# Kotomiya07/kuzushiji-vision

Hardware: AMD Instinct MI355X
Metric: line-images/sec (train) (higher is better)
Workload: dtype bf16; 1 GPU; TrOCR train step: ViT-B/16 (12L/768/12h/3072) on 64x640 crops (S_e=161) + RoBERTa decoder 6L/256/4h/768, V=4300 one-char vocab, labels [B,128], dropout 0.1, clip 1.0, RAdamScheduleFree; BASELINE.json configs[1]; per_gpu_batch=256, global_batch=256, parallelism=dp1

## Files before the change

### include/kzv.h

```cpp
#ifndef KZV_H
#define KZV_H
#include <stddef.h>
#include <stdint.h>

#ifdef __cplusplus
extern "C" {
#endif

#define KZV_OK 0
#define KZV_E_ARG (-1)
#define KZV_E_HIP (-2)
#define KZV_E_STATE (-3)

const char* kzv_last_error(void);
int kzv_version(void);

typedef struct kzv_config {
    int32_t image_h, image_w, patch_h, patch_w, channels;
    int32_t enc_hidden, enc_layers, enc_heads, enc_ffn;
    int32_t dec_hidden, dec_layers, dec_heads, dec_ffn;
    int32_t vocab, max_pos, type_vocab, pad_id;
    float enc_hidden_dropout, enc_attn_dropout, dec_hidden_dropout, dec_attn_dropout;
    float ln_eps;
} kzv_config;
// ... 206 lines not shown
    void* c8; int64_t ldc8;
    const float* c8_qscale; float* c8_amax;
    int32_t M, N, K, n_valid;
    float drop_p; uint32_t drop_key;
    const float* c8_rowq;
} kzv_gemm_nt_fp8_args;
int kzv_gemm_nt_fp8(const kzv_gemm_nt_fp8_args* a, int epilogue, void* stream);
int kzv_quant_rows_fp8(const float* x, int64_t rows, int64_t cols, void* q, float* scale, void* stream);
int kzv_layernorm_fwd_fp8(const float* x, const float* gamma, const float* beta, void* y_bf16, void* y_fp8, float* y_scale,
                          float* stats, int rows, int H, float eps, void* stream);
int kzv_set_fp8(kzv_model* m, int mode);
int kzv_get_fp8(const kzv_model* m);
int kzv_fp8_act_scales(const kzv_model* m, float* d_out, void* stream);

typedef struct kzv_gemm_tn_args {
    const void* P; int64_t ldp;
    const void* Q; int64_t ldq;
    float* OUT; int64_t ldo;
    int32_t Mtok, N, K, n_store;
    float* dbias;
} kzv_gemm_tn_args;
int kzv_gemm_tn(const kzv_gemm_tn_args* a, void* stream);

int kzv_gemm_dgrad_wgrad(const kzv_gemm_nt_args* nt, int epilogue, const kzv_gemm_tn_args* tn, void* stream);
int kzv_set_pair(int on);

int kzv_gemm_nt_f32(const kzv_gemm_nt_args* a, int epilogue, void* stream);
int kzv_gemm_tn_f32(const kzv_gemm_tn_args* a, void* stream);

int kzv_layernorm_fwd(const float* x, const float* gamma, const float* beta, void* y_bf16, float* y_f32,
                      float* stats , int rows, int H, float eps, void* stream);
int kzv_layernorm_bwd(const void* dy, int dy_is_f32, const float* x, const float* stats, const float* gamma,
                      float* dx, int accumulate_dx, float* dgamma, float* dbeta, int rows, int H, void* stream);
typedef struct kzv_ln_fwd_args {
    const float* x; const float* gamma; const float* beta;
    void* y_bf16; float* y_f32;
    float* stats;
    int32_t rows, H, seq, drop_first;
    float eps, drop_p; uint32_t drop_key;
} kzv_ln_fwd_args;
int kzv_ln_fwd_ex(const kzv_ln_fwd_args* a, void* stream);
typedef struct kzv_ln_bwd_args {
    const void* dy; const float* x; const float* stats; const float* gamma;
    float* dx; float* dgamma; float* dbeta;
    void* out16;
    int32_t dy_is_f32, accumulate_dx, rows, H, seq, drop_first;
// ... 150 lines not shown
```

### kuzushiji-vision_amd/csrc/gemm.hip

```cpp
#include "kzv_common.h"
#include "../../include/kzv.h"
#include "kzv_host.h"
#include "gemm_nt.h"
#include "gemm_tn.h"

namespace {

constexpr int BK = 64;
constexpr int STAGE_BYTES = (128 + 128) * BK * 2;
constexpr int NT_LDS = 2 * STAGE_BYTES;

template <int N> __device__ __forceinline__ void wait_vmcnt() {
    if constexpr (N == 0) asm volatile("s_waitcnt vmcnt(0)" ::: "memory");
    else if constexpr (N == 4) asm volatile("s_waitcnt vmcnt(4)" ::: "memory");
    else if constexpr (N == 6) asm volatile("s_waitcnt vmcnt(6)" ::: "memory");
    else if constexpr (N == 8) asm volatile("s_waitcnt vmcnt(8)" ::: "memory");
    else if constexpr (N == 12) asm volatile("s_waitcnt vmcnt(12)" ::: "memory");
    else if constexpr (N == 16) asm volatile("s_waitcnt vmcnt(16)" ::: "memory");
    else static_assert(N == 0, "add the vmcnt literal");
}

template <int EPI, int WM, int WN, int NSTAGE, int KB, bool ASM_DMA>
__global__ __launch_bounds__(WM * WN * 64) void gemm_nt_kernel(const NtParams p) {
    constexpr int BM = WM * 64, BN = WN * 64, NW = WM * WN;
// ... 280 lines not shown
    const bool interior = tnb * 128 + 128 <= p.n_store && tkb * 128 + 128 <= p.K;
    for (int it0 = 0; it0 < 64; it0 += 8) {
        float v[8];
#pragma unroll
        for (int u = 0; u < 8; ++u) {
            const int it = it0 + u;
            const int n = w * 32 + (it >> 1), k = (it & 1) * 64 + lane;
            v[u] = tile[n * 128 + ((((k >> 2) ^ (n & 31)) << 2) | (k & 3))];
        }
#pragma unroll
        for (int u = 0; u < 8; ++u) {
            const int it = it0 + u;
            const int n = w * 32 + (it >> 1), k = (it & 1) * 64 + lane;
            const int gn = tnb * 128 + n, gk = tkb * 128 + k;
            float* o = p.OUT + (int64_t)gn * p.ldo + gk;
            if (interior && p.splits > 1) atomicAdd(o, v[u]);
            else if (gn < p.n_store && gk < p.K) { if (p.splits == 1) *o += v[u]; else atomicAdd(o, v[u]); }
        }
    }
}

__global__ __launch_bounds__(256, 2) void gemm_tn_kernel(const TnParams p) { gemm_tn_body(p, blockIdx.x); }

constexpr int TN_GROUP_MAX = 40;
struct TnGroup { TnParams p[TN_GROUP_MAX]; int start[TN_GROUP_MAX + 1]; int n; };
__global__ __launch_bounds__(256, 2) void gemm_tn_group_kernel(const TnGroup g) {
    int i = 0;
#pragma unroll 1
    while (i + 1 < g.n && (int)blockIdx.x >= g.start[i + 1]) ++i;
    gemm_tn_body(g.p[i], (int)blockIdx.x - g.start[i]);
}

}

static int g_nt_schedule = -1;
static int g_nt_half_mask = -1;
static int nt_schedule() {
    if (g_nt_schedule < 0) {
        g_nt_schedule = kzv_env_int("KZV_NT_FREE", 0) != 0;
        if (kzv_env_int("KZV_NT_HALF", 0)) g_nt_schedule |= 2;
    }
    return g_nt_schedule;
}
static int nt_half_mask() {
    if (g_nt_half_mask < 0) g_nt_half_mask = kzv_env_int("KZV_NT_HALF_EPIS", 0x3f);
    return g_nt_half_mask;
}
extern "C" int kzv_set_nt_schedule(int n) { g_nt_schedule = n < 0 ? -1 : (n & 3); return KZV_OK; }
// ... 126 lines not shown
    if (splits < 1) splits = 1;
    const int chunk_tiles = (tok_tiles + splits - 1) / splits;
    splits = (tok_tiles + chunk_tiles - 1) / chunk_tiles;
    p.splits = splits; p.chunk = chunk_tiles * 64;
    return tiles * splits;
}
static int tn_target() {
    static int target = -1;
    if (target < 0) target = kzv_env_int("KZV_TN_BLOCKS", 512);
    return target;
}

extern "C" int kzv_gemm_tn(const kzv_gemm_tn_args* a, void* stream) {
    TnParams p;
    const int rc = tn_fill(a, p);
    if (rc != KZV_OK) return rc;
    KzvProfScope prof(1, 2.0 * a->Mtok * p.n_store * a->K, (hipStream_t)stream);
    if (kzv_tn256_launch(p, (hipStream_t)stream)) return kzv_check_launch("gemm_tn");
    const int blocks = tn_plan(p, tn_target());
    kzv_launch_lds<gemm_tn_kernel>(dim3(blocks), dim3(256), NT_LDS, (hipStream_t)stream, p);
    return kzv_check_launch("gemm_tn");
}

int kzv_gemm_tn_group(const kzv_gemm_tn_args* a, int n, hipStream_t s) {
    if (n <= 0) return KZV_OK;
    if (n == 1 || n > TN_GROUP_MAX) {
        for (int i = 0; i < n; ++i) { const int rc = kzv_gemm_tn(a + i, s); if (rc != KZV_OK) return rc; }
        return KZV_OK;
    }
    TnGroup g;
    g.n = 0;
    int tiles_total = 0;
    double work = 0;
    for (int i = 0; i < n; ++i) {
        TnParams p;
        const int rc = tn_fill(a + i, p);
        if (rc != KZV_OK) return rc;
        const int t256 = ((p.n_store + 255) / 256) * ((p.K + 255) / 256);
        if (t256 >= 24) { const int r2 = kzv_gemm_tn(a + i, s); if (r2 != KZV_OK) return r2; continue; }
        g.p[g.n++] = p;
        tiles_total += ((p.N + 127) / 128) * ((p.K + 127) / 128);
        work += 2.0 * p.Mtok * p.n_store * p.K;
    }
    if (g.n == 0) return KZV_OK;
    KzvProfScope prof(1, work, s);
    int blocks = 0;
    for (int i = 0; i < g.n; ++i) {
        const int tiles = ((g.p[i].N + 127) / 128) * ((g.p[i].K + 127) / 128);
        const int target = tiles_total >= 256 ? 2 * tn_target() : tn_target();
        int share = (int)((int64_t)target * tiles / tiles_total);
        if (share < tiles) share = tiles;
        g.start[i] = blocks;
        blocks += tn_plan(g.p[i], share);
    }
    g.start[g.n] = blocks;
    kzv_launch_lds<gemm_tn_group_kernel>(dim3(blocks), dim3(256), NT_LDS, s, g);
    return kzv_check_launch("gemm_tn_group");
}
```

### kuzushiji-vision_amd/csrc/gemm_tn.h

```cpp
#pragma once
#include "kzv_common.h"

struct TnParams {
    const bf16_t* P; const bf16_t* Q; float* OUT; const void* zero16;
    int64_t ldp, ldq, ldo;
    int Mtok, N, K, n_store, splits, chunk;
    float* dbias;
};

inline bool tn_dma_offsets_fit(const TnParams& p) {
    return (uint64_t)64 * (uint64_t)p.ldp * 2 + (uint64_t)p.N * 2 <= 0xffffffffull && (uint64_t)64 * (uint64_t)p.ldq * 2 + (uint64_t)p.K * 2 <= 0xffffffffull;
}

int kzv_tn256_launch(const TnParams& p, hipStream_t s);

struct KzvTnFoldScope { explicit KzvTnFoldScope(hipStream_t stream); ~KzvTnFoldScope(); hipStream_t s; };

struct kzv_gemm_nt_args; struct kzv_gemm_tn_args;
int kzv_gemm_pair_launch(const kzv_gemm_nt_args* na, int epilogue, const kzv_gemm_tn_args* ta, hipStream_t s);
```

### kuzushiji-vision_amd/csrc/gemm_tn256.hip

```cpp
#include "kzv_common.h"
#include "../../include/kzv.h"
#include "kzv_host.h"
#include "gemm_tn.h"
#include "gemm_nt.h"
#include "gemm256_common.h"
#include "gemm_nt256p_body.h"
#include <vector>
#include <type_traits>

namespace {

constexpr int HT_BYTES = 64 * 256;
constexpr int BUF_BYTES = 4 * HT_BYTES;
constexpr int LDS_BYTES = 2 * BUF_BYTES;
constexpr int KP0 = 0, KP1 = 1, KQ0 = 2, KQ1 = 3;
#ifndef KZV_TN_F32_PARTIALS
constexpr size_t PART_FLOATS = 32768;
#else
constexpr size_t PART_FLOATS = 65536;
#endif

__global__ __launch_bounds__(512) void gemm_tn256_kernel(const TnParams p, float* part_ws) {
    extern __shared__ __attribute__((aligned(16))) char smem[];
    const int tid = threadIdx.x, lane = tid & 63;
    const int w = __builtin_amdgcn_readfirstlane(tid >> 6);
    const int g = lane >> 4, l15 = lane & 15;
    const int wr = w >> 2, wc = w & 3;
    const int tilesN = (p.N + 255) / 256, tilesK = (p.K + 255) / 256;
    const int per = tilesN * tilesK;
    const int id = xcd_remap(blockIdx.x, per * p.splits);
    const int split = id / per, rem = id - split * per;
    const int tnb = rem / tilesK, tkb = rem - tnb * tilesK;
    const int t_begin = split * p.chunk;
    const int t_end = min(p.Mtok, t_begin + p.chunk);
    const int nt = (t_end - t_begin) >> 6;

    const char* baseP = (const char*)(p.P + (int64_t)t_begin * p.ldp);
    const char* baseQ = (const char*)(p.Q + (int64_t)t_begin * p.ldq);
    const int64_t stepP = 64 * p.ldp * 2, stepQ = 64 * p.ldq * 2;
    unsigned voff[4][2];
#pragma unroll
    for (int j = 0; j < 2; ++j) {
        const int r = (w + 8 * j) * 4 + (lane >> 4);
// ... 115 lines not shown

    stage(0, KP0, 0); stage(0, KQ0, 0); stage(0, KQ1, 0); stage(0, KP1, 0); stage(1, KP0, 1); stage(1, KQ0, 1);
    vmcnt<8>();
    __builtin_amdgcn_s_barrier();
    if (wr == 1) __builtin_amdgcn_s_barrier();
    for (int t = 0; t < nt; t += 2) {
        ktile(I0{}, t);
        if (t + 1 < nt) ktile(I1{}, t + 1);
    }
    if (wr == 0) __builtin_amdgcn_s_barrier();

    if (bias_wave) {
#pragma unroll
        for (int j = 0; j < 8; ++j) {
            float v = bsum[j];
            v += __shfl_xor(v, 16, 64);
            v += __shfl_xor(v, 32, 64);
            const int n = tnb * 256 + (j >> 2) * 128 + wr * 64 + (j & 3) * 16 + l15;
            if (g == 0 && n < p.n_store) atomicAdd(p.dbias + n, v);
        }
    }

    float* tile = (float*)smem;
    float* part = part_ws + (size_t)id * PART_FLOATS;
#pragma unroll
    for (int c = 0; c < 2; ++c) {
        __syncthreads();
#pragma unroll
        for (int j = 0; j < 4; ++j)
#pragma unroll
            for (int i = 0; i < 4; ++i)
#pragma unroll
                for (int r = 0; r < 4; ++r) {
                    const int ln = wr * 64 + j * 16 + 4 * g + r;
                    const int k = (i >> 1) * 128 + wc * 32 + (i & 1) * 16 + l15;
                    tile[ln * 256 + ((((k >> 2) ^ (ln & 31)) << 2) | (k & 3))] = acc[i][c * 4 + j][r];
                }
        __syncthreads();
#pragma unroll
        for (int it = 0; it < 16; ++it) {
            const int ln = w * 16 + it;
            const f32x4 v = *(const f32x4*)(tile + ln * 256 + ((lane ^ (ln & 31)) << 2));
            const int row = c * 128 + ln;
#ifndef KZV_TN_F32_PARTIALS
            typedef __attribute__((ext_vector_type(2))) unsigned u32x2p;
            __builtin_nontemporal_store((u32x2p){pack_bf2(v[0], v[1]), pack_bf2(v[2], v[3])}, (u32x2p*)((bf16_t*)part + row * 256 + lane * 4));
#else
            __builtin_nontemporal_store(v, (f32x4*)(part + row * 256 + lane * 4));
#endif
        }
    }
}

__device__ __forceinline__ void tn256f_body(const TnParams& p, float* const part, const int tnb, const int tkb, const int t_begin, const int nt,
                                            char* const smem) {
    const int tid = threadIdx.x, lane = tid & 63;
    const int w = __builtin_amdgcn_readfirstlane(tid >> 6);
    const int g = lane >> 4, l15 = lane & 15;
    const int wr = w >> 2, wc = w & 3;
    const int tilesK = (p.K + 255) / 256;

    const unsigned ldp2 = (unsigned)p.ldp * 2u, ldq2 = (unsigned)p.ldq * 2u;
    const char* baseP = (const char*)(p.P + (int64_t)t_begin * p.ldp);
    const char* baseQ = (const char*)(p.Q + (int64_t)t_begin * p.ldq);
    const int64_t stepP = 64 * (int64_t)ldp2, stepQ = 64 * (int64_t)ldq2;
    unsigned cP[2], cQ[2];
    {
        const int r = w * 4 + (lane >> 4);
        const int col2 = ((lane & 15) ^ ((r & 7) << 1)) * 16;
#pragma unroll
        for (int h = 0; h < 2; ++h) {
            cP[h] = (unsigned)r * ldp2 + (unsigned)min((tnb * 256 + h * 128) * 2 + col2, (p.N - 8) * 2);
            cQ[h] = (unsigned)r * ldq2 + (unsigned)min((tkb * 256 + h * 128) * 2 + col2, (p.K - 8) * 2);
        }
    }
    const unsigned ldsw = __builtin_amdgcn_readfirstlane((unsigned)(__SIZE_TYPE__)((KZV_LDS char*)smem) + (unsigned)w * 1024u);
// ... 133 lines not shown
            if (g == 0 && n < p.n_store) atomicAdd(p.dbias + n, v);
        }
    }

    float* tile = (float*)smem;
#pragma unroll
    for (int c = 0; c < 2; ++c) {
        __syncthreads();
#pragma unroll
        for (int j = 0; j < 4; ++j)
#pragma unroll
            for (int i = 0; i < 4; ++i)
#pragma unroll
                for (int r = 0; r < 4; ++r) {
                    const int ln = wr * 64 + j * 16 + 4 * g + r;
                    const int k = (i >> 1) * 128 + wc * 32 + (i & 1) * 16 + l15;
                    tile[ln * 256 + ((((k >> 2) ^ (ln & 31)) << 2) | (k & 3))] = acc[i][c * 4 + j][r];
                }
        __syncthreads();
#pragma unroll
        for (int it = 0; it < 16; ++it) {
            const int ln = w * 16 + it;
            const f32x4 v = *(const f32x4*)(tile + ln * 256 + ((lane ^ (ln & 31)) << 2));
            const int row = c * 128 + ln;
#ifndef KZV_TN_F32_PARTIALS
            typedef __attribute__((ext_vector_type(2))) unsigned u32x2p;
            __builtin_nontemporal_store((u32x2p){pack_bf2(v[0], v[1]), pack_bf2(v[2], v[3])}, (u32x2p*)((bf16_t*)part + row * 256 + lane * 4));
#else
            __builtin_nontemporal_store(v, (f32x4*)(part + row * 256 + lane * 4));
#endif
        }
    }
}

__global__ __launch_bounds__(512) void gemm_tn256f_kernel(const TnParams p, float* part_ws) {
    extern __shared__ __attribute__((aligned(16))) char smem[];
    const int tilesN = (p.N + 255) / 256, tilesK = (p.K + 255) / 256;
    const int per = tilesN * tilesK;
    const int id = xcd_remap(blockIdx.x, per * p.splits);
    const int split = id / per, rem = id - split * per;
    const int t_begin = split * p.chunk;
    const int t_end = min(p.Mtok, t_begin + p.chunk);
    tn256f_body(p, part_ws + (size_t)id * PART_FLOATS, rem / tilesK, rem % tilesK, t_begin, (t_end - t_begin) >> 6, smem);
}

struct PairPlan { unsigned short tile[256], split[256], t0[256], cnt[256]; };

template <int EPI>
__global__ __launch_bounds__(512) void gemm_pair_kernel(const NtParams pn, const int tiles, const int tilesN, const int strip_in, const TnParams pt,
                                                        float* part_ws, const int per, const PairPlan plan) {
    extern __shared__ __attribute__((aligned(16))) char smem[];
    nt256p_body<EPI, false>(pn, tiles, tilesN, strip_in, (int)blockIdx.x, (int)gridDim.x, smem);
    const int cnt = plan.cnt[blockIdx.x];
    if (cnt == 0) return;
    __syncthreads();
    const int tile = plan.tile[blockIdx.x], split = plan.split[blockIdx.x];
    const int tilesK = (pt.K + 255) / 256;
    tn256f_body(pt, part_ws + ((size_t)split * per + tile) * PART_FLOATS, tile / tilesK, tile % tilesK, (int)plan.t0[blockIdx.x] * 64, cnt, smem);
}

__global__ __launch_bounds__(256) void gemm_tn256_fold_kernel(const float* part_ws, float* OUT, int64_t ldo, int n_store, int K,
                                                             int tilesK, int per, int splits) {
    const int tile = blockIdx.x >> 6;
    const int row = (blockIdx.x & 63) * 4 + (threadIdx.x >> 6), k4 = (threadIdx.x & 63) * 4;
    const int tnb = tile / tilesK, tkb = tile - tnb * tilesK;
    const int gn = tnb * 256 + row, gk = tkb * 256 + k4;
    if (gn >= n_store || gk >= K) return;
    f32x4 s = (f32x4){0.f, 0.f, 0.f, 0.f};
#ifndef KZV_TN_F32_PARTIALS
    typedef __attribute__((ext_vector_type(2))) unsigned u32x2p;
#pragma unroll 4
    for (int sp = 0; sp < splits; ++sp) {
        const u32x2p u = __builtin_nontemporal_load((const u32x2p*)((const bf16_t*)(part_ws + ((size_t)sp * per + tile) * PART_FLOATS) + row * 256 + k4));
        s[0] += bf2f((bf16_t)(u[0] & 0xffffu)); s[1] += bf2f((bf16_t)(u[0] >> 16)); s[2] += bf2f((bf16_t)(u[1] & 0xffffu)); s[3] += bf2f((bf16_t)(u[1] >> 16));
    }
#else
    const float* src = part_ws + ((size_t)tile * 256 + row) * 256 + k4;
#pragma unroll 4
    for (int sp = 0; sp < splits; ++sp) s += __builtin_nontemporal_load((const f32x4*)(src + (size_t)sp * per * PART_FLOATS));
#endif
    f32x4* o = (f32x4*)(OUT + (int64_t)gn * ldo + gk);
    *o += s;
}

constexpr int TN_REGIONS = 6;
KzvScratch g_tn_buf;
size_t g_tn_region = 0;
float* tn_partials(size_t floats, int region) {
    const size_t stride = floats > g_tn_region ? floats : g_tn_region;
    float* base = (float*)g_tn_buf.get((size_t)TN_REGIONS * stride * sizeof(float));
    if (!base) return nullptr;
    g_tn_region = stride;
    return base + (size_t)region * stride;
}

struct TnFold { const float* ws; float* OUT; int64_t ldo; int n_store, K, tilesK, per, splits, block0; };
struct TnFoldTable { TnFold e[TN_REGIONS - 1]; int n; };
__global__ __launch_bounds__(256) void gemm_tn256_fold_multi_kernel(const TnFoldTable t) {
    int k = 0;
    while (k + 1 < t.n && (int)blockIdx.x >= t.e[k + 1].block0) ++k;
    const TnFold& e = t.e[k];
    const int bid = blockIdx.x - e.block0;
    const int tile = bid >> 6;
    const int row = (bid & 63) * 4 + (threadIdx.x >> 6), k4 = (threadIdx.x & 63) * 4;
    const int tnb = tile / e.tilesK, tkb = tile - tnb * e.tilesK;
    const int gn = tnb * 256 + row, gk = tkb * 256 + k4;
    if (gn >= e.n_store || gk >= e.K) return;
    f32x4 s = (f32x4){0.f, 0.f, 0.f, 0.f};
#ifndef KZV_TN_F32_PARTIALS
    typedef __attribute__((ext_vector_type(2))) unsigned u32x2p;
#pragma unroll 4
    for (int sp = 0; sp < e.splits; ++sp) {
        const u32x2p u = __builtin_nontemporal_load((const u32x2p*)((const bf16_t*)(e.ws + ((size_t)sp * e.per + tile) * PART_FLOATS) + row * 256 + k4));
        s[0] += bf2f((bf16_t)(u[0] & 0xffffu)); s[1] += bf2f((bf16_t)(u[0] >> 16)); s[2] += bf2f((bf16_t)(u[1] & 0xffffu)); s[3] += bf2f((bf16_t)(u[1] >> 16));
    }
#else
    const float* src = e.ws + ((size_t)tile * 256 + row) * 256 + k4;
#pragma unroll 4
    for (int sp = 0; sp < e.splits; ++sp) s += __builtin_nontemporal_load((const f32x4*)(src + (size_t)sp * e.per * PART_FLOATS));
#endif
    f32x4* o = (f32x4*)(e.OUT + (int64_t)gn * e.ldo + gk);
    *o += s;
}
int g_tn_defer = 0;
std::vector<TnFold> g_tn_pending;
int tn_flush(hipStream_t s) {
    if (g_tn_pending.empty()) return KZV_OK;
    TnFoldTable t;
    int blocks = 0;
    for (size_t i = 0; i < g_tn_pending.size(); ++i) { t.e[i] = g_tn_pending[i]; t.e[i].block0 = blocks; blocks += g_tn_pending[i].per * 64; }
    t.n = (int)g_tn_pending.size();
    hipLaunchKernelGGL(gemm_tn256_fold_multi_kernel, dim3(blocks), dim3(256), 0, s, t);
    g_tn_pending.clear();
    return kzv_check_launch("gemm_tn256_fold");
}

int g_tn_schedule = -1;
int tn_schedule() {
    if (g_tn_schedule < 0) g_tn_schedule = kzv_env_int("KZV_TN_FREE", 1) != 0;
    return g_tn_schedule;
}
int tn256_min_tiles() {
    static int v = -1;
    if (v < 0) v = kzv_env_int("KZV_TN256_MIN_TILES", 9);
    return v;
}

}

int kzv_tn256_launch(const TnParams& p0, hipStream_t s) {
    const int tiles = ((p0.N + 255) / 256) * ((p0.K + 255) / 256);
    const int tok_tiles = p0.Mtok / 64;
    if (tiles < tn256_min_tiles() || p0.Mtok % 64 || tok_tiles < 2 || p0.N < 8 || p0.K < 8) return 0;
    if (!tn_dma_offsets_fit(p0)) return 0;
    TnParams p = p0;
    int cus = kzv_device_cus() - kzv_cu_reserve();
    { const int g = kzv_env_int("KZV_TN_CUS", 0); if (g > 0 && g < cus) cus = g; }
    int splits = cus / tiles;
    if (splits > tok_tiles / 8) splits = tok_tiles / 8;
    if (splits < 1) splits = 1;
    int chunk_tiles = (tok_tiles + splits - 1) / splits;
    if (chunk_tiles < 2) chunk_tiles = 2;
    splits = (tok_tiles + chunk_tiles - 1) / chunk_tiles;
    if (tok_tiles - (splits - 1) * chunk_tiles < 2) return 0;
    p.splits = splits; p.chunk = chunk_tiles * 64;
    if (p.K % 4 || p.ldo % 4 || ((uintptr_t)p.OUT & 15)) return 0;
    const size_t need = (size_t)tiles * splits * PART_FLOATS;
    const bool deferred = g_tn_defer > 0;
    bool same_out = false;
    for (const TnFold& e : g_tn_pending) same_out |= e.OUT == p.OUT;
    if (deferred && ((int)g_tn_pending.size() == TN_REGIONS - 1 || need > g_tn_region || same_out)) {
        if (tn_flush(s) != KZV_OK) return 0;
    }
    float* ws = tn_partials(need, deferred ? 1 + (int)g_tn_pending.size() : 0);
    if (!ws) return 0;
    if (tn_schedule()) kzv_launch_lds<gemm_tn256f_kernel>(dim3(tiles * splits), dim3(512), LDS_BYTES, s, p, ws);
    else kzv_launch_lds<gemm_tn256_kernel>(dim3(tiles * splits), dim3(512), LDS_BYTES, s, p, ws);
    if (deferred) {
        g_tn_pending.push_back(TnFold{ws, p.OUT, p.ldo, p.n_store, p.K, (p.K + 255) / 256, tiles, splits, 0});
        return 1;
    }
    hipLaunchKernelGGL(gemm_tn256_fold_kernel, dim3(tiles * 64), dim3(256), 0, s, ws, p.OUT, p.ldo, p.n_store, p.K,
                       (p.K + 255) / 256, tiles, splits);
    return 1;
}

int kzv_nt_params(const kzv_gemm_nt_args* a, int epilogue, NtParams* out);

namespace {
int g_pair = -1;
int pair_enabled() {
    if (g_pair < 0) g_pair = kzv_env_int("KZV_PAIR", 0) != 0;
    return g_pair;
}
double pair_ratio(int nk, int epilogue) {
    static int ov = -2;
    if (ov == -2) ov = kzv_env_int("KZV_PAIR_R", -1);
    const double drain = (epilogue == KZV_EPI_DGELU || epilogue == KZV_EPI_RESID) ? 5.0 : 2.5;
    const double r = 0.6 * (nk * 1.45 + drain) / 1.55;
    return ov >= 0 ? r * ov * 0.01 / 0.6 : r;
}
}

int kzv_gemm_pair_launch(const kzv_gemm_nt_args* na, int epilogue, const kzv_gemm_tn_args* ta, hipStream_t s) {
    if (!pair_enabled() || kzv_cu_reserve() != 0 || !tn_schedule() || kzv_device_cus() != 256) return 0;
    if (epilogue != KZV_EPI_BF16 && epilogue != KZV_EPI_F32 && epilogue != KZV_EPI_DGELU && epilogue != KZV_EPI_RESID) return 0;
    NtParams pn;
    if (kzv_nt_params(na, epilogue, &pn) != KZV_OK) return 0;
// ... 31 lines not shown
    std::vector<int> t0((size_t)tilesNw * S), cnt((size_t)tilesNw * S);
    for (int tn = 0; tn < tilesNw; ++tn) {
        double csum = 0;
        for (int sp = 0; sp < S; ++sp) csum += cg[(size_t)tn * S + sp];
        const double level = (stages + r * csum) / S;
        double acc = 0; int prev = 0;
        for (int sp = 0; sp < S; ++sp) {
            double n = level - r * cg[(size_t)tn * S + sp];
            if (n < 2) n = 2;
            acc += n;
            int end = sp == S - 1 ? stages : (int)(acc + 0.5);
            const int left = S - 1 - sp;
            if (end > stages - 2 * left) end = stages - 2 * left;
            if (end < prev + 2) end = prev + 2;
            t0[(size_t)tn * S + sp] = prev; cnt[(size_t)tn * S + sp] = end - prev; prev = end;
        }
        if (prev != stages) return 0;
    }
    for (int b = 0; b < nwg; ++b) {
        const int sp = idb[b] / per, tl = idb[b] % per; const size_t gi = (size_t)(tl / tilesKw) * S + sp;
        plan.tile[b] = (unsigned short)tl; plan.split[b] = (unsigned short)sp; plan.t0[b] = (unsigned short)t0[gi]; plan.cnt[b] = (unsigned short)cnt[gi];
    }
    pt.splits = S; pt.chunk = 0;
    const size_t need = (size_t)per * S * PART_FLOATS;
    const bool deferred = g_tn_defer > 0;
    bool same_out = false;
    for (const TnFold& e : g_tn_pending) same_out |= e.OUT == pt.OUT;
    if (deferred && ((int)g_tn_pending.size() == TN_REGIONS - 1 || need > g_tn_region || same_out)) {
        if (tn_flush(s) != KZV_OK) return 0;
    }
    float* ws = tn_partials(need, deferred ? 1 + (int)g_tn_pending.size() : 0);
    if (!ws) return 0;
    KzvProfScope prof(5, 2.0 * pn.M * pn.n_valid * pn.K + 2.0 * pt.Mtok * pt.N * pt.K, s);
#define KZV_PAIR_CASE(E) case E: kzv_launch_lds<gemm_pair_kernel<E>>(dim3(G), dim3(512), NT256P_LDS_BYTES, s, pn, tiles, tilesN, kzv_nt_strip(), pt, ws, per, plan); break;
    switch (epilogue) {
        KZV_PAIR_CASE(KZV_EPI_BF16) KZV_PAIR_CASE(KZV_EPI_F32) KZV_PAIR_CASE(KZV_EPI_DGELU) KZV_PAIR_CASE(KZV_EPI_RESID)
        default: return 0;
    }
#undef KZV_PAIR_CASE
    if (deferred) g_tn_pending.push_back(TnFold{ws, pt.OUT, pt.ldo, pt.n_store, pt.K, tilesKw, per, S, 0});
    else hipLaunchKernelGGL(gemm_tn256_fold_kernel, dim3(per * 64), dim3(256), 0, s, ws, pt.OUT, pt.ldo, pt.n_store, pt.K, tilesKw, per, S);
    return kzv_check_launch("gemm_pair") == KZV_OK ? 1 : -1;
}

extern "C" int kzv_set_pair(int n) { g_pair = n < 0 ? -1 : (n != 0); return KZV_OK; }
extern "C" int kzv_gemm_dgrad_wgrad(const kzv_gemm_nt_args* na, int epilogue, const kzv_gemm_tn_args* ta, void* stream) {
    if (!na || !ta) return kzv_fail(KZV_E_ARG, "gemm_dgrad_wgrad: null");
// ... 11 lines not shown
```

### kuzushiji-vision_amd/csrc/kzv_kernels.h

```cpp
#pragma once
#include <hip/hip_runtime.h>
#include <stdint.h>
#include "kzv_common.h"

int kzv_ln_fwd_ex(const float* x, const float* gamma, const float* beta, void* y16, float* y32, float* stats,
                  int rows, int H, float eps, int seq, int drop_first, float drop_p, uint32_t drop_key, hipStream_t s,
                  void* y8 = nullptr, float* y8_scale = nullptr);
struct KzvLnBwdF8 { void* out8; float* scale; float* rq; float* rqinv; const float* wnorm; };
int kzv_ln_bwd_ex(const void* dy, int dy_is_f32, const float* x, const float* stats, const float* gamma, float* dx,
                  int accumulate_dx, float* dgamma, float* dbeta, int rows, int H, int seq, int drop_first,
                  float drop_p, uint32_t drop_key, hipStream_t s, bf16_t* out16 = nullptr, float out_drop_p = 0.f,
                  uint32_t out_drop_key = 0, const KzvLnBwdF8* f8 = nullptr);

struct KzvLnDeferScope { explicit KzvLnDeferScope(hipStream_t stream); ~KzvLnDeferScope(); hipStream_t s; };

constexpr int KZV_LN_SLOTS = 32;
float* kzv_ln_partial_region(float* dgamma, float* dbeta, int H, hipStream_t s, bool* fold_now);
int kzv_ln_partial_fold(float* partial, float* dgamma, float* dbeta, int H, hipStream_t s);

int kzv_im2row(const float* px, bf16_t* out, int B, int C, int H, int W, int ph, int pw, hipStream_t s);
int kzv_embed_assemble(const float* patch_emb, const float* cls, const float* pos, float* x0, int B, int np, int He,
                       float drop_p, uint32_t key, hipStream_t s, int gw = 0, int gw_max = 0);
int kzv_embed_assemble_bwd(const float* dx0, bf16_t* dpatch, float* dcls, float* dpos, float* dpatch_bias, int B, int np,
                           int He, float drop_p, uint32_t key, hipStream_t s, int gw = 0, int gw_max = 0);
// ... 4 lines not shown
int kzv_embed_gather(const int64_t* labels, int L, const int* posids, const float* word, const float* type0,
                     const float* postab, float* out, int B, int T, int Hd, hipStream_t s);
int kzv_embed_scatter_bwd(const float* dsum, const int64_t* labels, int L, const int* posids, float* dword, float* dtype0,
                          float* dpostab, int B, int T, int Hd, int pad, hipStream_t s);
int kzv_ce_fwd_bwd(const float* logits, int64_t ldl, const int64_t* labels, int L, int B, int T, int V, int pad,
                   const float* count, float* loss, bf16_t* dlogits, hipStream_t s);
int kzv_copy_logits(const float* logits, int64_t ldl, float* out, int rows, int V, hipStream_t s);

struct KzvCastDesc {
    const float* src; bf16_t* dst; bf16_t* dstT;
    int rows, cols; int64_t ldT; int tile0, tiles_c;
};
int kzv_cast_weights(const KzvCastDesc* d_desc, int ndesc, int total_tiles, hipStream_t s);

struct KzvQuantDesc {
    const float* src; unsigned char* dst; float* scale; int rows, cols, row0;
    const bf16_t* src16; int64_t ld16;
    float* normmax;
};
int kzv_quant_rows(const KzvQuantDesc* d_desc, int ndesc, int total_rows, hipStream_t s);
int kzv_fp8_roll(float* qscale, float* amax, float* row_scales, int sites, int rows, hipStream_t s);

struct kzv_gemm_tn_args;
int kzv_gemm_tn_group(const kzv_gemm_tn_args* a, int n, hipStream_t s);

int kzv_sqnorm(const float* g, int64_t n, float* out1, float* scratch, hipStream_t s);


int kzv_attn_decode(const bf16_t* q, int64_t ldq, const bf16_t* knew, const bf16_t* vnew, int64_t ldnew, bf16_t* K, bf16_t* V, int64_t kb,
                    int64_t kj, const unsigned char* valid, int64_t ldvalid, bf16_t* out, int64_t ldo, int B, int heads, int nkeys,
                    int append_at, hipStream_t s, const int* tptr = nullptr, int group = 1, int* rows = nullptr, int64_t ldrows = 0, int64_t kh = 64);
int kzv_kv_rows(const int* src, int* dst, const int64_t* parent, int B, int ld, int len, hipStream_t s);
int kzv_step_inc(int* d_t, hipStream_t s);
int kzv_cross_relayout(const bf16_t* src, bf16_t* dst, int images, int keys, int heads, int layers2, hipStream_t s);
int kzv_cross_relayout_pool(const bf16_t* src, bf16_t* dst, int images, int keys, int heads, int layers2, int dst_images, int first, hipStream_t s);

#define KZV_DECODE_FUSED_MAX_LAYERS 12
struct KzvDecodeFusedLayer {
    const bf16_t *wqkv, *wo, *wcq, *wco, *wfc1, *wfc2;
    const float *bqkv, *bo, *bcq, *bco, *bfc1, *bfc2;
    const float *ln1w, *ln1b, *ln2w, *ln2b, *ln3w, *ln3b;
};
struct KzvDecodeFused {
    KzvDecodeFusedLayer layers[KZV_DECODE_FUSED_MAX_LAYERS]; int nlayers;
    const int64_t* tokens; const int* posids;
    const float *word, *type0, *postab, *elnw, *elnb;
    const bf16_t* whd; const float* bhd; float* hd_out;
// ... 45 lines not shown
```

### kuzushiji-vision_amd/kzv/_lib.py

```python
from __future__ import annotations

import ctypes as C
import os

_HERE = os.path.dirname(os.path.abspath(__file__))
LIB_PATH = os.environ.get("KZV_LIB") or os.path.join(_HERE, "libkzv.so")


class KzvError(RuntimeError):
    pass


class kzv_config(C.Structure):
    _fields_ = [(n, C.c_int32) for n in (
        "image_h", "image_w", "patch_h", "patch_w", "channels",
        "enc_hidden", "enc_layers", "enc_heads", "enc_ffn",
        "dec_hidden", "dec_layers", "dec_heads", "dec_ffn",
        "vocab", "max_pos", "type_vocab", "pad_id")] + [(n, C.c_float) for n in (
        "enc_hidden_dropout", "enc_attn_dropout", "dec_hidden_dropout", "dec_attn_dropout", "ln_eps")]


class kzv_opt_step(C.Structure):
    _fields_ = [("lr_t", C.c_float), ("ckp1", C.c_float), ("beta1", C.c_float), ("beta2", C.c_float),
                ("eps", C.c_float), ("weight_decay", C.c_float), ("bias_correction2", C.c_float),
# ... 151 lines not shown
    "kzv_zero_grads": (C.c_int, [_P, _P]),
    "kzv_backward_segments": (C.c_int, [_P]),
    "kzv_backward_segment": (C.c_int, [_P, C.c_int, _P]),
    "kzv_backward_segment_range": (C.c_int, [_P, C.c_int, C.POINTER(C.c_int64), C.POINTER(C.c_int64)]),
    "kzv_backward": (C.c_int, [_P, _P]),
    "kzv_grad_sqnorm": (C.c_int, [_P, C.c_int64, _P, _P, _P]),
    "kzv_clip_and_step": (C.c_int, [_P, _P, _P, _P, C.c_int64, _P, C.POINTER(kzv_opt_step), _P]),
    "kzv_clip_and_step_ema": (C.c_int, [_P, _P, _P, _P, C.c_int64, _P, C.POINTER(kzv_opt_step), _P, C.c_float, _P]),
    "kzv_lerp_params": (C.c_int, [_P, _P, C.c_int64, C.c_float, _P]),
    "kzv_gemm_nt": (C.c_int, [C.POINTER(kzv_gemm_nt_args), C.c_int, _P]),
    "kzv_set_rows_max_m": (C.c_int, [C.c_int]),
    "kzv_set_nt_schedule": (C.c_int, [C.c_int]),
    "kzv_set_nt_half_epilogues": (C.c_int, [C.c_int]),
    "kzv_set_nt_half_stagger": (C.c_int, [C.c_int]),
    "kzv_set_tn_schedule": (C.c_int, [C.c_int]),
    "kzv_gemm_rows_ln": (C.c_int, [C.POINTER(kzv_gemm_rows_ln_args), C.c_int, _P]),
    "kzv_gemm_nt_fp8": (C.c_int, [C.POINTER(kzv_gemm_nt_fp8_args), C.c_int, _P]),
    "kzv_quant_rows_fp8": (C.c_int, [_P, C.c_int64, C.c_int64, _P, _P, _P]),
    "kzv_layernorm_fwd_fp8": (C.c_int, [_P, _P, _P, _P, _P, _P, _P, C.c_int, C.c_int, C.c_float, _P]),
    "kzv_set_fp8": (C.c_int, [_P, C.c_int]),
    "kzv_get_fp8": (C.c_int, [_P]),
    "kzv_fp8_act_scales": (C.c_int, [_P, _P, _P]),
    "kzv_gemm_tn": (C.c_int, [C.POINTER(kzv_gemm_tn_args), _P]),
    "kzv_layernorm_fwd": (C.c_int, [_P, _P, _P, _P, _P, _P, C.c_int, C.c_int, C.c_float, _P]),
    "kzv_layernorm_bwd": (C.c_int, [_P, C.c_int, _P, _P, _P, _P, C.c_int, _P, _P, C.c_int, C.c_int, _P]),
    "kzv_ln_fwd_ex": (C.c_int, [C.POINTER(kzv_ln_fwd_args), _P]),
    "kzv_ln_bwd_ex": (C.c_int, [C.POINTER(kzv_ln_bwd_args), _P]),
    "kzv_im2row": (C.c_int, [_P, _P] + [C.c_int] * 6 + [_P]),
    "kzv_embed_assemble": (C.c_int, [_P, _P, _P, _P, C.c_int, C.c_int, C.c_int, C.c_float, C.c_uint32, C.c_int, C.c_int, _P]),
    "kzv_embed_assemble_bwd": (C.c_int, [_P, _P, _P, _P, _P, C.c_int, C.c_int, C.c_int, C.c_float, C.c_uint32, C.c_int, C.c_int, _P]),
    "kzv_cast_drop_colsum": (C.c_int, [_P, _P, _P, C.c_int, C.c_int, C.c_float, C.c_uint32, _P, _P]),
    "kzv_colsum_bf16": (C.c_int, [_P, C.c_int64, _P, C.c_int, C.c_int, _P]),
    "kzv_dec_prepare": (C.c_int, [_P] + [C.c_int] * 5 + [_P, _P, _P, _P]),
    "kzv_embed_gather": (C.c_int, [_P, C.c_int, _P, _P, _P, _P, _P, C.c_int, C.c_int, C.c_int, _P]),
    "kzv_embed_scatter_bwd": (C.c_int, [_P, _P, C.c_int, _P, _P, _P, _P, C.c_int, C.c_int, C.c_int, C.c_int, _P]),
    "kzv_ce_fwd_bwd": (C.c_int, [_P, C.c_int64, _P] + [C.c_int] * 5 + [_P, _P, _P, _P]),
    "kzv_copy_logits": (C.c_int, [_P, C.c_int64, _P, C.c_int, C.c_int, _P]),
    "kzv_cast_weights": (C.c_int, [C.POINTER(kzv_cast_desc), C.c_int, _P]),
    "kzv_attn_fwd": (C.c_int, [C.POINTER(kzv_attn_args), _P]),
    "kzv_attn_bwd": (C.c_int, [C.POINTER(kzv_attn_args), _P]),
    "kzv_attn_impl": (C.c_int, [C.POINTER(kzv_attn_args), C.c_int]),
    "kzv_attn_stream_fwd": (C.c_int, [C.POINTER(kzv_attn_args), _P]),
    "kzv_attn_stream_bwd": (C.c_int, [C.POINTER(kzv_attn_args), _P]),
    "kzv_attn_impl_ex": (C.c_int, [C.POINTER(kzv_attn_args), C.c_int, C.c_uint]),
    "kzv_attn_probs": (C.c_int, [C.POINTER(kzv_attn_probs_args), _P]),
    "kzv_token_scores": (C.c_int, [_P, C.c_int64, _P, C.c_int64, C.c_int, C.c_int, C.c_int, C.c_int, _P, _P, _P, _P]),
# ... 141 lines not shown
```

Baseline: 8524 img/s.

## Route grouped small TN weight-grad GEMMs through a split-K 256-tile grouped kernel

Adds a grouped 256x256-tile TN (weight-gradient) kernel with split-token partials and a grouped fold. Small wgrad GEMMs that previously went to the 128-tile group kernel are packed into one launch sized to the CU budget, with f32 partials reduced by a follow-up fold kernel. Entries that write to the same output are split off and launched separately. This is meant to raise utilization for many small wgrad GEMMs, at the cost of extra partial-buffer traffic, a second kernel launch, and workspace memory. It is enabled by default through an environment flag and is also exported through the C API and Python bindings.

Result: no change. 8547 img/s (median of 6 runs) (+0.3%).

```diff
diff --git a/include/kzv.h b/include/kzv.h
--- a/include/kzv.h
+++ b/include/kzv.h
@@ -252,6 +252,9 @@
 } kzv_gemm_tn_args;
 int kzv_gemm_tn(const kzv_gemm_tn_args* a, void* stream);
 
+int kzv_gemm_tn_batch(const kzv_gemm_tn_args* a, int n, void* stream);
+int kzv_set_tn_group256(int on);
+
 int kzv_gemm_dgrad_wgrad(const kzv_gemm_nt_args* nt, int epilogue, const kzv_gemm_tn_args* tn, void* stream);
 int kzv_set_pair(int on);
 
diff --git a/kuzushiji-vision_amd/csrc/gemm.hip b/kuzushiji-vision_amd/csrc/gemm.hip
--- a/kuzushiji-vision_amd/csrc/gemm.hip
+++ b/kuzushiji-vision_amd/csrc/gemm.hip
@@ -326,8 +326,6 @@
 
 __global__ __launch_bounds__(256, 2) void gemm_tn_kernel(const TnParams p) { gemm_tn_body(p, blockIdx.x); }
 
-constexpr int TN_GROUP_MAX = 40;
-struct TnGroup { TnParams p[TN_GROUP_MAX]; int start[TN_GROUP_MAX + 1]; int n; };
 __global__ __launch_bounds__(256, 2) void gemm_tn_group_kernel(const TnGroup g) {
     int i = 0;
 #pragma unroll 1
@@ -500,7 +498,7 @@
     return kzv_check_launch("gemm_tn");
 }
 
-int kzv_gemm_tn_group(const kzv_gemm_tn_args* a, int n, hipStream_t s) {
+extern "C" int kzv_gemm_tn_group(const kzv_gemm_tn_args* a, int n, hipStream_t s) {
     if (n <= 0) return KZV_OK;
     if (n == 1 || n > TN_GROUP_MAX) {
         for (int i = 0; i < n; ++i) { const int rc = kzv_gemm_tn(a + i, s); if (rc != KZV_OK) return rc; }
@@ -508,7 +506,6 @@
     }
     TnGroup g;
     g.n = 0;
-    int tiles_total = 0;
     double work = 0;
     for (int i = 0; i < n; ++i) {
         TnParams p;
@@ -517,11 +514,31 @@
         const int t256 = ((p.n_store + 255) / 256) * ((p.K + 255) / 256);
         if (t256 >= 24) { const int r2 = kzv_gemm_tn(a + i, s); if (r2 != KZV_OK) return r2; continue; }
         g.p[g.n++] = p;
-        tiles_total += ((p.N + 127) / 128) * ((p.K + 127) / 128);
         work += 2.0 * p.Mtok * p.n_store * p.K;
     }
     if (g.n == 0) return KZV_OK;
     KzvProfScope prof(1, work, s);
+    {
+        unsigned char taken[TN_GROUP_MAX];
+        KZV_TRY_RC(kzv_tn256_group_launch(g.p, g.n, taken, s));
+        int kept = 0;
+        for (int i = 0; i < g.n; ++i) if (!taken[i]) g.p[kept++] = g.p[i];
+        g.n = kept;
+    }
+    if (g.n == 0) return KZV_OK;
+    TnParams repeats[TN_GROUP_MAX];
+    int n_repeats = 0;
+    {
+        int kept = 0;
+        for (int i = 0; i < g.n; ++i) {
+            bool same_out = false;
+            for (int j = 0; j < kept; ++j) same_out |= g.p[j].OUT == g.p[i].OUT;
+            if (same_out) repeats[n_repeats++] = g.p[i]; else g.p[kept++] = g.p[i];
+        }
+        g.n = kept;
+    }
+    int tiles_total = 0;
+    for (int i = 0; i < g.n; ++i) tiles_total += ((g.p[i].N + 127) / 128) * ((g.p[i].K + 127) / 128);
     int blocks = 0;
     for (int i = 0; i < g.n; ++i) {
         const int tiles = ((g.p[i].N + 127) / 128) * ((g.p[i].K + 127) / 128);
@@ -533,5 +550,14 @@
     }
     g.start[g.n] = blocks;
     kzv_launch_lds<gemm_tn_group_kernel>(dim3(blocks), dim3(256), NT_LDS, s, g);
+    for (int i = 0; i < n_repeats; ++i) {
+        const int b = tn_plan(repeats[i], tn_target());
+        kzv_launch_lds<gemm_tn_kernel>(dim3(b), dim3(256), NT_LDS, s, repeats[i]);
+    }
     return kzv_check_launch("gemm_tn_group");
 }
+
+extern "C" int kzv_gemm_tn_batch(const kzv_gemm_tn_args* a, int n, void* stream) {
+    if (n < 0 || (n > 0 && !a)) return kzv_fail(KZV_E_ARG, "gemm_tn_batch: null or negative count");
+    return kzv_gemm_tn_group(a, n, (hipStream_t)stream);
+}
diff --git a/kuzushiji-vision_amd/csrc/gemm_tn.h b/kuzushiji-vision_amd/csrc/gemm_tn.h
--- a/kuzushiji-vision_amd/csrc/gemm_tn.h
+++ b/kuzushiji-vision_amd/csrc/gemm_tn.h
@@ -12,6 +12,11 @@
     return (uint64_t)64 * (uint64_t)p.ldp * 2 + (uint64_t)p.N * 2 <= 0xffffffffull && (uint64_t)64 * (uint64_t)p.ldq * 2 + (uint64_t)p.K * 2 <= 0xffffffffull;
 }
 
+constexpr int TN_GROUP_MAX = 40;
+struct TnGroup { TnParams p[TN_GROUP_MAX]; int start[TN_GROUP_MAX + 1]; int n; };
+
+int kzv_tn256_group_launch(const TnParams* p, int n, unsigned char* taken, hipStream_t s);
+
 int kzv_tn256_launch(const TnParams& p, hipStream_t s);
 
 struct KzvTnFoldScope { explicit KzvTnFoldScope(hipStream_t stream); ~KzvTnFoldScope(); hipStream_t s; };
diff --git a/kuzushiji-vision_amd/csrc/gemm_tn256.hip b/kuzushiji-vision_amd/csrc/gemm_tn256.hip
--- a/kuzushiji-vision_amd/csrc/gemm_tn256.hip
+++ b/kuzushiji-vision_amd/csrc/gemm_tn256.hip
@@ -14,11 +14,40 @@
 constexpr int BUF_BYTES = 4 * HT_BYTES;
 constexpr int LDS_BYTES = 2 * BUF_BYTES;
 constexpr int KP0 = 0, KP1 = 1, KQ0 = 2, KQ1 = 3;
+enum TnPart { TN_PART_BF16 = 0, TN_PART_F32 = 1 };
 #ifndef KZV_TN_F32_PARTIALS
-constexpr size_t PART_FLOATS = 32768;
+constexpr TnPart TN_PART = TN_PART_BF16;
 #else
-constexpr size_t PART_FLOATS = 65536;
+constexpr TnPart TN_PART = TN_PART_F32;
 #endif
+template <TnPart F> constexpr size_t PART_FLOATS = F == TN_PART_F32 ? 65536 : 32768;
+
+template <TnPart F>
+__device__ __forceinline__ void part_store(float* part, int row, int lane, const f32x4 v) {
+    if constexpr (F == TN_PART_BF16) {
+        typedef __attribute__((ext_vector_type(2))) unsigned u32x2p;
+        __builtin_nontemporal_store((u32x2p){pack_bf2(v[0], v[1]), pack_bf2(v[2], v[3])}, (u32x2p*)((bf16_t*)part + row * 256 + lane * 4));
+    } else {
+        __builtin_nontemporal_store(v, (f32x4*)(part + row * 256 + lane * 4));
+    }
+}
+template <TnPart F>
+__device__ __forceinline__ f32x4 part_sum(const float* ws, int tile, int row, int k4, int per, int splits) {
+    f32x4 s = (f32x4){0.f, 0.f, 0.f, 0.f};
+    if constexpr (F == TN_PART_BF16) {
+        typedef __attribute__((ext_vector_type(2))) unsigned u32x2p;
+#pragma unroll 4
+        for (int sp = 0; sp < splits; ++sp) {
+            const u32x2p u = __builtin_nontemporal_load((const u32x2p*)((const bf16_t*)(ws + ((size_t)sp * per + tile) * PART_FLOATS<F>) + row * 256 + k4));
+            s[0] += bf2f((bf16_t)(u[0] & 0xffffu)); s[1] += bf2f((bf16_t)(u[0] >> 16)); s[2] += bf2f((bf16_t)(u[1] & 0xffffu)); s[3] += bf2f((bf16_t)(u[1] >> 16));
+        }
+    } else {
+        const float* src = ws + ((size_t)tile * 256 + row) * 256 + k4;
+#pragma unroll 4
+        for (int sp = 0; sp < splits; ++sp) s += __builtin_nontemporal_load((const f32x4*)(src + (size_t)sp * per * PART_FLOATS<F>));
+    }
+    return s;
+}
 
 __global__ __launch_bounds__(512) void gemm_tn256_kernel(const TnParams p, float* part_ws) {
     extern __shared__ __attribute__((aligned(16))) char smem[];
@@ -180,7 +209,7 @@
     }
 
     float* tile = (float*)smem;
-    float* part = part_ws + (size_t)id * PART_FLOATS;
+    float* part = part_ws + (size_t)id * PART_FLOATS<TN_PART>;
 #pragma unroll
     for (int c = 0; c < 2; ++c) {
         __syncthreads();
@@ -199,17 +228,12 @@
         for (int it = 0; it < 16; ++it) {
             const int ln = w * 16 + it;
             const f32x4 v = *(const f32x4*)(tile + ln * 256 + ((lane ^ (ln & 31)) << 2));
-            const int row = c * 128 + ln;
-#ifndef KZV_TN_F32_PARTIALS
-            typedef __attribute__((ext_vector_type(2))) unsigned u32x2p;
-            __builtin_nontemporal_store((u32x2p){pack_bf2(v[0], v[1]), pack_bf2(v[2], v[3])}, (u32x2p*)((bf16_t*)part + row * 256 + lane * 4));
-#else
-            __builtin_nontemporal_store(v, (f32x4*)(part + row * 256 + lane * 4));
-#endif
-        }
-    }
-}
-
+            part_store<TN_PART>(part, c * 128 + ln, lane, v);
+        }
+    }
+}
+
+template <TnPart F>
 __device__ __forceinline__ void tn256f_body(const TnParams& p, float* const part, const int tnb, const int tkb, const int t_begin, const int nt,
                                             char* const smem) {
     const int tid = threadIdx.x, lane = tid & 63;
@@ -389,13 +413,7 @@
         for (int it = 0; it < 16; ++it) {
             const int ln = w * 16 + it;
             const f32x4 v = *(const f32x4*)(tile + ln * 256 + ((lane ^ (ln & 31)) << 2));
-            const int row = c * 128 + ln;
-#ifndef KZV_TN_F32_PARTIALS
-            typedef __attribute__((ext_vector_type(2))) unsigned u32x2p;
-            __builtin_nontemporal_store((u32x2p){pack_bf2(v[0], v[1]), pack_bf2(v[2], v[3])}, (u32x2p*)((bf16_t*)part + row * 256 + lane * 4));
-#else
-            __builtin_nontemporal_store(v, (f32x4*)(part + row * 256 + lane * 4));
-#endif
+            part_store<F>(part, c * 128 + ln, lane, v);
         }
     }
 }
@@ -408,7 +426,23 @@
     const int split = id / per, rem = id - split * per;
     const int t_begin = split * p.chunk;
     const int t_end = min(p.Mtok, t_begin + p.chunk);
-    tn256f_body(p, part_ws + (size_t)id * PART_FLOATS, rem / tilesK, rem % tilesK, t_begin, (t_end - t_begin) >> 6, smem);
+    tn256f_body<TN_PART>(p, part_ws + (size_t)id * PART_FLOATS<TN_PART>, rem / tilesK, rem % tilesK, t_begin, (t_end - t_begin) >> 6, smem);
+}
+
+__global__ __launch_bounds__(512) void gemm_tn256f_group_kernel(const TnGroup g, float* part_ws) {
+    extern __shared__ __attribute__((aligned(16))) char smem[];
+    const int id = xcd_remap(blockIdx.x, g.start[g.n]);
+    int i = 0;
+#pragma unroll 1
+    while (i + 1 < g.n && id >= g.start[i + 1]) ++i;
+    const TnParams& p = g.p[i];
+    const int tilesN = (p.N + 255) / 256, tilesK = (p.K + 255) / 256;
+    const int per = tilesN * tilesK;
+    const int lid = id - g.start[i];
+    const int split = lid / per, rem = lid - split * per;
+    const int t_begin = split * p.chunk;
+    const int t_end = min(p.Mtok, t_begin + p.chunk);
+    tn256f_body<TN_PART_F32>(p, part_ws + (size_t)id * PART_FLOATS<TN_PART_F32>, rem / tilesK, rem % tilesK, t_begin, (t_end - t_begin) >> 6, smem);
 }
 
 struct PairPlan { unsigned short tile[256], split[256], t0[256], cnt[256]; };
@@ -423,7 +457,7 @@
     __syncthreads();
     const int tile = plan.tile[blockIdx.x], split = plan.split[blockIdx.x];
     const int tilesK = (pt.K + 255) / 256;
-    tn256f_body(pt, part_ws + ((size_t)split * per + tile) * PART_FLOATS, tile / tilesK, tile % tilesK, (int)plan.t0[blockIdx.x] * 64, cnt, smem);
+    tn256f_body<TN_PART>(pt, part_ws + ((size_t)split * per + tile) * PART_FLOATS<TN_PART>, tile / tilesK, tile % tilesK, (int)plan.t0[blockIdx.x] * 64, cnt, smem);
 }
 
 __global__ __launch_bounds__(256) void gemm_tn256_fold_kernel(const float* part_ws, float* OUT, int64_t ldo, int n_store, int K,
@@ -433,21 +467,8 @@
     const int tnb = tile / tilesK, tkb = tile - tnb * tilesK;
     const int gn = tnb * 256 + row, gk = tkb * 256 + k4;
     if (gn >= n_store || gk >= K) return;
-    f32x4 s = (f32x4){0.f, 0.f, 0.f, 0.f};
-#ifndef KZV_TN_F32_PARTIALS
-    typedef __attribute__((ext_vector_type(2))) unsigned u32x2p;
-#pragma unroll 4
-    for (int sp = 0; sp < splits; ++sp) {
-        const u32x2p u = __builtin_nontemporal_load((const u32x2p*)((const bf16_t*)(part_ws + ((size_t)sp * per + tile) * PART_FLOATS) + row * 256 + k4));
-        s[0] += bf2f((bf16_t)(u[0] & 0xffffu)); s[1] += bf2f((bf16_t)(u[0] >> 16)); s[2] += bf2f((bf16_t)(u[1] & 0xffffu)); s[3] += bf2f((bf16_t)(u[1] >> 16));
-    }
-#else
-    const float* src = part_ws + ((size_t)tile * 256 + row) * 256 + k4;
-#pragma unroll 4
-    for (int sp = 0; sp < splits; ++sp) s += __builtin_nontemporal_load((const f32x4*)(src + (size_t)sp * per * PART_FLOATS));
-#endif
     f32x4* o = (f32x4*)(OUT + (int64_t)gn * ldo + gk);
-    *o += s;
+    *o += part_sum<TN_PART>(part_ws, tile, row, k4, per, splits);
 }
 
 constexpr int TN_REGIONS = 6;
@@ -462,8 +483,9 @@
 }
 
 struct TnFold { const float* ws; float* OUT; int64_t ldo; int n_store, K, tilesK, per, splits, block0; };
-struct TnFoldTable { TnFold e[TN_REGIONS - 1]; int n; };
-__global__ __launch_bounds__(256) void gemm_tn256_fold_multi_kernel(const TnFoldTable t) {
+template <int MAXN> struct TnFoldTable { TnFold e[MAXN]; int n; };
+template <TnPart F, int MAXN>
+__device__ __forceinline__ void tn256_fold_multi(const TnFoldTable<MAXN>& t) {
     int k = 0;
     while (k + 1 < t.n && (int)blockIdx.x >= t.e[k + 1].block0) ++k;
     const TnFold& e = t.e[k];
@@ -473,27 +495,16 @@
     const int tnb = tile / e.tilesK, tkb = tile - tnb * e.tilesK;
     const int gn = tnb * 256 + row, gk = tkb * 256 + k4;
     if (gn >= e.n_store || gk >= e.K) return;
-    f32x4 s = (f32x4){0.f, 0.f, 0.f, 0.f};
-#ifndef KZV_TN_F32_PARTIALS
-    typedef __attribute__((ext_vector_type(2))) unsigned u32x2p;
-#pragma unroll 4
-    for (int sp = 0; sp < e.splits; ++sp) {
-        const u32x2p u = __builtin_nontemporal_load((const u32x2p*)((const bf16_t*)(e.ws + ((size_t)sp * e.per + tile) * PART_FLOATS) + row * 256 + k4));
-        s[0] += bf2f((bf16_t)(u[0] & 0xffffu)); s[1] += bf2f((bf16_t)(u[0] >> 16)); s[2] += bf2f((bf16_t)(u[1] & 0xffffu)); s[3] += bf2f((bf16_t)(u[1] >> 16));
-    }
-#else
-    const float* src = e.ws + ((size_t)tile * 256 + row) * 256 + k4;
-#pragma unroll 4
-    for (int sp = 0; sp < e.splits; ++sp) s += __builtin_nontemporal_load((const f32x4*)(src + (size_t)sp * e.per * PART_FLOATS));
-#endif
     f32x4* o = (f32x4*)(e.OUT + (int64_t)gn * e.ldo + gk);
-    *o += s;
-}
+    *o += part_sum<F>(e.ws, tile, row, k4, e.per, e.splits);
+}
+__global__ __launch_bounds__(256) void gemm_tn256_fold_multi_kernel(const TnFoldTable<TN_REGIONS - 1> t) { tn256_fold_multi<TN_PART>(t); }
+__global__ __launch_bounds__(256) void gemm_tn256_fold_group_kernel(const TnFoldTable<TN_GROUP_MAX> t) { tn256_fold_multi<TN_PART_F32>(t); }
 int g_tn_defer = 0;
 std::vector<TnFold> g_tn_pending;
 int tn_flush(hipStream_t s) {
     if (g_tn_pending.empty()) return KZV_OK;
-    TnFoldTable t;
+    TnFoldTable<TN_REGIONS - 1> t;
     int blocks = 0;
     for (size_t i = 0; i < g_tn_pending.size(); ++i) { t.e[i] = g_tn_pending[i]; t.e[i].block0 = blocks; blocks += g_tn_pending[i].per * 64; }
     t.n = (int)g_tn_pending.size();
@@ -532,7 +543,7 @@
     if (tok_tiles - (splits - 1) * chunk_tiles < 2) return 0;
     p.splits = splits; p.chunk = chunk_tiles * 64;
     if (p.K % 4 || p.ldo % 4 || ((uintptr_t)p.OUT & 15)) return 0;
-    const size_t need = (size_t)tiles * splits * PART_FLOATS;
+    const size_t need = (size_t)tiles * splits * PART_FLOATS<TN_PART>;
     const bool deferred = g_tn_defer > 0;
     bool same_out = false;
     for (const TnFold& e : g_tn_pending) same_out |= e.OUT == p.OUT;
@@ -551,6 +562,97 @@
                        (p.K + 255) / 256, tiles, splits);
     return 1;
 }
+
+namespace {
+int g_tn_group256 = -1;
+int tn_group256() {
+    if (g_tn_group256 < 0) g_tn_group256 = kzv_env_int("KZV_TN_GROUP256", 1) != 0;
+    return g_tn_group256;
+}
+KzvScratch g_tn_group_buf;
+
+bool tn_group_splits(int stages, int c, int* splits_out, int* chunk_out) {
+    int splits = (stages + c - 1) / c;
+    if (splits > stages / 8) splits = stages / 8;
+    if (splits < 1) splits = 1;
+    const int chunk = (stages + splits - 1) / splits;
+    splits = (stages + chunk - 1) / chunk;
+    *splits_out = splits; *chunk_out = chunk;
+    return stages - (splits - 1) * chunk >= 2;
+}
+
+int tn_group_issue(const TnParams* p, const int* idx, int m, int budget, unsigned char* taken, hipStream_t s) {
+    int64_t tile_stages = 0;
+    int max_stages = 2;
+    for (int j = 0; j < m; ++j) {
+        const TnParams& q = p[idx[j]];
+        const int stages = q.Mtok / 64;
+        tile_stages += (int64_t)((q.N + 255) / 256) * ((q.K + 255) / 256) * stages;
+        if (stages > max_stages) max_stages = stages;
+    }
+    int c = (int)((tile_stages + budget - 1) / budget);
+    if (c < 8) c = 8;
+    for (; c < max_stages; ++c) {
+        int blocks = 0;
+        for (int j = 0; j < m; ++j) {
+            const TnParams& q = p[idx[j]];
+            int splits, chunk;
+            (void)tn_group_splits(q.Mtok / 64, c, &splits, &chunk);
+            blocks += ((q.N + 255) / 256) * ((q.K + 255) / 256) * splits;
+        }
+        if (blocks <= budget) break;
+    }
+    TnGroup g;
+    TnFoldTable<TN_GROUP_MAX> f;
+    g.n = 0;
+    int blocks = 0, fold_blocks = 0;
+    for (int j = 0; j < m; ++j) {
+        TnParams q = p[idx[j]];
+        int splits, chunk;
+        if (!tn_group_splits(q.Mtok / 64, c, &splits, &chunk)) continue;
+        const int tilesK = (q.K + 255) / 256, per = ((q.N + 255) / 256) * tilesK;
+        q.splits = splits; q.chunk = chunk * 64;
+        g.p[g.n] = q; g.start[g.n] = blocks;
+        f.e[g.n] = TnFold{nullptr, q.OUT, q.ldo, q.n_store, q.K, tilesK, per, splits, fold_blocks};
+        blocks += per * splits; fold_blocks += per * 64;
+        ++g.n;
+        taken[idx[j]] = 1;
+    }
+    if (g.n == 0) return KZV_OK;
+    g.start[g.n] = blocks;
+    f.n = g.n;
+    float* ws = (float*)g_tn_group_buf.get((size_t)blocks * PART_FLOATS<TN_PART_F32> * sizeof(float));
+    if (!ws) return kzv_fail(KZV_E_HIP, "gemm_tn_group: partial-tile workspace");
+    for (int i = 0; i < g.n; ++i) f.e[i].ws = ws + (size_t)g.start[i] * PART_FLOATS<TN_PART_F32>;
+    kzv_launch_lds<gemm_tn256f_group_kernel>(dim3(blocks), dim3(512), LDS_BYTES, s, g, ws);
+    hipLaunchKernelGGL(gemm_tn256_fold_group_kernel, dim3(fold_blocks), dim3(256), 0, s, f);
+    return kzv_check_launch("gemm_tn256_group");
+}
+}
+
+int kzv_tn256_group_launch(const TnParams* p, int n, unsigned char* taken, hipStream_t s) {
+    for (int i = 0; i < n; ++i) taken[i] = 0;
+    if (!tn_group256() || n > TN_GROUP_MAX) return KZV_OK;
+    const int budget = kzv_device_cus() - kzv_cu_reserve();
+    int idx[TN_GROUP_MAX], m = 0, tiles = 0;
+    for (int i = 0; i < n; ++i) {
+        const TnParams& q = p[i];
+        if (q.Mtok % 64 || q.Mtok < 128 || q.N < 8 || q.K < 8 || !tn_dma_offsets_fit(q)) continue;
+        if (q.K % 4 || q.ldo % 4 || ((uintptr_t)q.OUT & 15)) continue;
+        const int t = ((q.N + 255) / 256) * ((q.K + 255) / 256);
+        if (t > budget) continue;
+        bool same_out = false;
+        for (int j = 0; j < i; ++j) same_out |= p[j].OUT == q.OUT;
+        if (same_out) continue;
+        if (tiles + t > budget) {
+            KZV_TRY_RC(tn_group_issue(p, idx, m, budget, taken, s));
+            m = 0; tiles = 0;
+        }
+        idx[m++] = i; tiles += t;
+    }
+    return m ? tn_group_issue(p, idx, m, budget, taken, s) : KZV_OK;
+}
+extern "C" int kzv_set_tn_group256(int on) { g_tn_group256 = on < 0 ? -1 : (on != 0); return KZV_OK; }
 
 int kzv_nt_params(const kzv_gemm_nt_args* a, int epilogue, NtParams* out);
 
@@ -628,7 +730,7 @@
         plan.tile[b] = (unsigned short)tl; plan.split[b] = (unsigned short)sp; plan.t0[b] = (unsigned short)t0[gi]; plan.cnt[b] = (unsigned short)cnt[gi];
     }
     pt.splits = S; pt.chunk = 0;
-    const size_t need = (size_t)per * S * PART_FLOATS;
+    const size_t need = (size_t)per * S * PART_FLOATS<TN_PART>;
     const bool deferred = g_tn_defer > 0;
     bool same_out = false;
     for (const TnFold& e : g_tn_pending) same_out |= e.OUT == pt.OUT;
diff --git a/kuzushiji-vision_amd/csrc/kzv_kernels.h b/kuzushiji-vision_amd/csrc/kzv_kernels.h
--- a/kuzushiji-vision_amd/csrc/kzv_kernels.h
+++ b/kuzushiji-vision_amd/csrc/kzv_kernels.h
@@ -50,7 +50,7 @@
 int kzv_fp8_roll(float* qscale, float* amax, float* row_scales, int sites, int rows, hipStream_t s);
 
 struct kzv_gemm_tn_args;
-int kzv_gemm_tn_group(const kzv_gemm_tn_args* a, int n, hipStream_t s);
+extern "C" int kzv_gemm_tn_group(const kzv_gemm_tn_args* a, int n, hipStream_t s);
 
 int kzv_sqnorm(const float* g, int64_t n, float* out1, float* scratch, hipStream_t s);
 
diff --git a/kuzushiji-vision_amd/kzv/_lib.py b/kuzushiji-vision_amd/kzv/_lib.py
--- a/kuzushiji-vision_amd/kzv/_lib.py
+++ b/kuzushiji-vision_amd/kzv/_lib.py
@@ -197,6 +197,9 @@
     "kzv_get_fp8": (C.c_int, [_P]),
     "kzv_fp8_act_scales": (C.c_int, [_P, _P, _P]),
     "kzv_gemm_tn": (C.c_int, [C.POINTER(kzv_gemm_tn_args), _P]),
+    "kzv_gemm_tn_batch": (C.c_int, [C.POINTER(kzv_gemm_tn_args), C.c_int, _P]),
+    "kzv_gemm_tn_group": (C.c_int, [C.POINTER(kzv_gemm_tn_args), C.c_int, _P]),
+    "kzv_set_tn_group256": (C.c_int, [C.c_int]),
     "kzv_layernorm_fwd": (C.c_int, [_P, _P, _P, _P, _P, _P, C.c_int, C.c_int, C.c_float, _P]),
     "kzv_layernorm_bwd": (C.c_int, [_P, C.c_int, _P, _P, _P, _P, C.c_int, _P, _P, C.c_int, C.c_int, _P]),
     "kzv_ln_fwd_ex": (C.c_int, [C.POINTER(kzv_ln_fwd_args), _P]),
```
